# wittyseok/multimodal-organ-segmentation

Hardware: AMD Instinct MI355X
Metric: 96^3 2-modality patches/sec/node (train step) (higher is better)
Workload: dtype bf16; 1 GPU; DualEncoder fusion=cross_attention (mean, dual_encoder.py:193-195) 96^3, modalities CT+PET, 6 classes, DiceCE, AdamW, per-GPU batch 2; model=dual_encoder, global_batch=2, parallelism=dp1, kernels=hip, tag=c3

## Files before the change

multimodal-organ-segmentation_amd/csrc/conv_gemm.hip:

```cpp
#include "mmseg_common.h"

#include <stdlib.h>

#include <algorithm>
#include <type_traits>
#include <cstdio>
#include <vector>

namespace {

int knob(const char* name, int dflt) {
  const char* v = getenv(name);
  return v ? atoi(v) : dflt;
}

enum GatherMode { MODE_CONV3 = 0, MODE_POINT = 1, MODE_CONVT_FWD = 2, MODE_CONVT_DGRAD = 3 };

#ifdef MMSEG_TIMING_PROBES
constexpr int PROBE_NB = 16384;
__device__ long long* g_probe = nullptr;
__device__ __forceinline__ void probe_block(bool end) {
  long long* p = g_probe;
  if (p && threadIdx.x == 0 && blockIdx.x < PROBE_NB) {
    p += 8LL * blockIdx.x;
// ... 1801 lines not shown
  int kind;
  int bz, by, bx;
  int ks;
  int bn;
};

Conv3Plan plan_conv3(int M, int Ncols, int cin, int D, int H, int W, int lda, int ldo, int tsize,
                     bool force_r = false) {
  Conv3Plan p{0, 0, 0, 0, 1, 32};
  bool k1_ok = false;
  const int brick = knob("MMSEG_BRICK", 2);
  const bool base_ok = cin % CK == 0 && lda % 8 == 0 && ldo % 8 == 0 && Ncols % 32 == 0;
  const bool ok48 = cin % CK == 0 && lda % 8 == 0 && ldo % 8 == 0 && Ncols % 48 == 0;
  if (!force_r && brick == 2 && (base_ok || ok48) && D % 4 == 0 && H % B2_Y == 0 && W % B2_X == 0) {
    const long long units = (long long)(M / (D * H * W)) * (D / 4) * (H / B2_Y) * (W / B2_X) *
                            ((Ncols + 63) / 64);
    if (!(base_ok && units < knob("MMSEG_BRICK2_MINUNITS", 128))) {
      p.kind = 1;
      return p;
    }
    k1_ok = true;
  }
  if (brick >= 2 && base_ok) {
    int best = 0;
    for (int bz = 1; bz <= D && bz <= 8; ++bz) {
      if (D % bz) continue;
      for (int by = 1; by <= H && by <= 16; ++by) {
        if (H % by) continue;
        for (int bx = 1; bx <= W && bx <= 16; ++bx) {
          if (W % bx) continue;
          const int rows = bz * by * bx;
          const int halo = (bz + 2) * (by + 2) * (bx + 2);
          const int hq = (bz + 2) * (by + 2) * ((bx + 2) * 2 * tsize + 2);
          if (rows > 256 || halo > BR_MAXHV || hq > br_xq(tsize)) continue;
          const int score = rows * 4 + (bx % 8 == 0 ? 2 : 0) + (by % 8 == 0 ? 1 : 0);
          const bool tie_better = score == best && halo < (p.bz + 2) * (p.by + 2) * (p.bx + 2);
          if (score > best || tie_better) {
            best = score;
            p.bz = bz; p.by = by; p.bx = bx;
          }
        }
      }
    }
    if (best >= 64 * 4) {
      p.kind = 2;
      p.bn = (tsize == 2 && Ncols % 64 == 0) ? 64 : 32;
      const int nb = (M / (D * H * W)) * (D / p.bz) * (H / p.by) * (W / p.bx);
      if (p.bn == 64 && nb * (Ncols / 64) < 256) p.bn = 32;
      const int nt = (Ncols + p.bn - 1) / p.bn;
      const int nchunk = cin / CK;
      const int slots = knob("MMSEG_BRICKR_SLOTS", 256);
      int ks = (slots + nb * nt - 1) / (nb * nt);
      if (ks > nchunk) ks = nchunk;
      if (ks < 1) ks = 1;
      const int cps = (nchunk + ks - 1) / ks;
      p.ks = (nchunk + cps - 1) / cps;
      return p;
    }
  }
  if (k1_ok) p.kind = 1;
  return p;
}

bool brick6_selected(const GemmArgs& g, int tsize) {
  if (tsize != 2 || g.ksplit != 1) return false;
  const Conv3Plan plan = plan_conv3(g.M, g.Ncols, 8 << g.cpg_shift, g.D, g.H, g.W, g.lda, g.ldo, tsize);
  if (plan.kind != 1) return false;
  const int nb1 = (g.M / (g.D * g.H * g.W)) * (g.D / 4) * (g.H / B2_Y) * (g.W / B2_X);
  const int min_blocks = knob("MMSEG_BRICK2_MINBLK", 512);
  const bool v3 = (long long)g.M * g.lda * 2LL < (1LL << 31);
  const bool wide = g.Ncols % 64 == 0 && nb1 * (g.Ncols / 64) >= min_blocks;
  if (!v3 || g.Ncols % 32 != 0 || gemm_nchunk(g) != 1 || wide) return false;
  return g.H % 4 == 0 && g.W % 16 == 0 && g.ldo % 8 == 0 && (reinterpret_cast<uintptr_t>(g.out) & 15) == 0;
}

inline bool tile_in_pitch(const GemmArgs& g, int BN) { return (long long)((g.Ncols + BN - 1) / BN) * BN <= g.Cpad; }
#define MMSEG_TILE(G, NAME, BN)                                                                                   \
  do {                                                                                                           \
    MMSEG_REQUIRE(tile_in_pitch((G), (BN)), "%s: %d-column tiles over %d columns exceed the packed pitch %d", \
                  (const char*)(NAME), (int)(BN), (G).Ncols, (G).Cpad);                                          \
    mmseg::note_kernel(NAME);                                                                                    \
  } while (0)

int launch_brick6(const GemmArgs& g, hipStream_t s) {
  const int nt_n = g.Ncols / 32;
  const int per_nt = std::max(1, knob("MMSEG_BRICK4_BLOCKS", 256) / nt_n);
  const int nb6 = (g.M / (g.D * g.H * g.W)) * (g.D / 4) * (g.H / 4) * (g.W / 16);
  const int upb6 = ceil_div(nb6, std::min(per_nt, nb6));
  const int bpn6 = ceil_div(nb6, upb6);
  const dim3 grid(bpn6 * nt_n), block(256);
  if (g.wdq) {
    MMSEG_TILE(g, "conv3_brick6_kernel<BN32,F8>", 32);
    if (g.nmean) MMSEG_LAUNCH((conv3_brick6_kernel<true, 6, false, true>), grid, block, 0, s, g, upb6, bpn6);
    else MMSEG_LAUNCH((conv3_brick6_kernel<false, 6, false, true>), grid, block, 0, s, g, upb6, bpn6);
    return upb6;
  }
  if (g.inpart) {
    MMSEG_TILE(g, "conv3_brick6_kernel<BN32,INP>", 32);
    MMSEG_LAUNCH((conv3_brick6_kernel<false, 6, true>), grid, block, 0, s, g, upb6, bpn6);
    return upb6;
  }
  MMSEG_TILE(g, "conv3_brick6_kernel<BN32>", 32);
  if (g.nmean)
    MMSEG_LAUNCH((conv3_brick6_kernel<true, 6>), grid, block, 0, s, g, upb6, bpn6);
  else
    MMSEG_LAUNCH((conv3_brick6_kernel<false, 6>), grid, block, 0, s, g, upb6, bpn6);
  return upb6;
}

template <int MODE>
__host__ __device__ __forceinline__ bool splitk_vec(const GemmArgs& g) {
  const bool al = (g.Ncols & 3) == 0 && (g.ldo & 3) == 0 && (reinterpret_cast<uintptr_t>(g.part) & 15) == 0;
  return MODE == MODE_CONVT_FWD ? al && ((g.Ncols >> 3) & 3) == 0 : al;
}
template <int MODE>
int splitk_reduce_blocks(const GemmArgs& g) {
  const long long total = (long long)g.M * g.Ncols;
  return ceil_div(splitk_vec<MODE>(g) ? (total + 3) / 4 : total, 256);
}

template <typename T, int MODE>
__global__ void gemm_splitk_reduce(GemmArgs g) {
  long long total = (long long)g.M * g.Ncols;
  if (MODE == MODE_CONVT_FWD && splitk_vec<MODE>(g)) {
    const long long idx4 = ((long long)blockIdx.x * blockDim.x + threadIdx.x) * 4;
    if (idx4 >= total) return;
    const long long row = idx4 / g.Ncols;
    const int col = (int)(idx4 - row * g.Ncols);
    const int Cout = g.Ncols >> 3, t = col / Cout, co = col - t * Cout;
    float4 v = make_float4(0.f, 0.f, 0.f, 0.f);
    const float4* p = reinterpret_cast<const float4*>(g.part + idx4);
    const long long st = total / 4;
#pragma unroll 4
    for (int k = 0; k < g.ksplit; ++k) {
      const float4 a = p[(long long)k * st];
      v.x += a.x; v.y += a.y; v.z += a.z; v.w += a.w;
    }
    if (g.bias) {
      v.x += g.bias[co]; v.y += g.bias[co + 1]; v.z += g.bias[co + 2]; v.w += g.bias[co + 3];
    }
    T* O = reinterpret_cast<T*>(g.out) + convt_child(row, t, g) * g.ldo + co;
    O[0] = from_f<T>(v.x); O[1] = from_f<T>(v.y); O[2] = from_f<T>(v.z); O[3] = from_f<T>(v.w);
    return;
  }
  if (MODE != MODE_CONVT_FWD && splitk_vec<MODE>(g)) {
    const long long idx4 = ((long long)blockIdx.x * blockDim.x + threadIdx.x) * 4;
    if (idx4 >= total) return;
    const long long row = idx4 / g.Ncols;
    const int col = (int)(idx4 - row * g.Ncols);
    float4 v = make_float4(0.f, 0.f, 0.f, 0.f);
    const float4* p = reinterpret_cast<const float4*>(g.part + idx4);
    const long long st = total / 4;
#pragma unroll 4
    for (int k = 0; k < g.ksplit; ++k) {
      const float4 a = p[(long long)k * st];
      v.x += a.x; v.y += a.y; v.z += a.z; v.w += a.w;
    }
    if (g.bias) {
      const float* bp = g.grp_n > 0 ? g.bias + (int)(row / ((long long)g.D * g.H * g.W) / g.grp_n) * g.b_gstride
                                    : g.bias;
      v.x += bp[col]; v.y += bp[col + 1]; v.z += bp[col + 2]; v.w += bp[col + 3];
    }
    T* O = out_at<T>(g, row, col);
    O[0] = from_f<T>(v.x); O[1] = from_f<T>(v.y); O[2] = from_f<T>(v.z); O[3] = from_f<T>(v.w);
    return;
  }
// ... 1524 lines not shown
      constexpr int PH = decltype(phc)::value;
      if (h_iss < h_tot) {
        issue(h_iss % WROW_NST, dq, du);
        dma_next();
        ++h_iss;
      }
      const char* S = ring + (h % WROW_NST) * WROW_SLOT;
      bf16x8 bfr[WROW_HY];
#pragma unroll
      for (int hy = 0; hy < WROW_HY; ++hy) {
        const bf16_t* pl = reinterpret_cast<const bf16_t*>(S + hy * (WROW_HX * 64) + boff);
        bfr[hy] = tr_frag(pl, pl + 8 * 32);
      }
      const bool anew = u < q.L;
      if (anew) {
#pragma unroll
        for (int r = 0; r < WROW_RY; ++r) {
          const bf16_t* pa = reinterpret_cast<const bf16_t*>(S + r * (32 * 64) + aoff);
          areg[PH][r] = tr_frag(pa, pa + 8 * 32);
        }
      }
      auto mm = [&](auto kzc, const bf16x8(&a)[WROW_RY]) __attribute__((always_inline)) {
        constexpr int KZ = decltype(kzc)::value;
#pragma unroll
        for (int hy = 0; hy < WROW_HY; ++hy)
#pragma unroll
          for (int ky = 0; ky < 3; ++ky) {
            const int ry = hy - ky;
            if (ry >= 0 && ry < WROW_RY)
              acc[KZ][ky] = __builtin_amdgcn_mfma_f32_16x16x32_bf16(a[ry], bfr[hy], acc[KZ][ky], 0, 0, 0);
          }
      };
      if (u >= 2) mm(std::integral_constant<int, 2>{}, areg[(PH + 1) % 3]);
      if (u >= 1 && u <= q.L) mm(std::integral_constant<int, 1>{}, areg[(PH + 2) % 3]);
      if (anew) {
        mm(std::integral_constant<int, 0>{}, areg[PH]);
        if (do_bias && h % 6 == kx * 2 + jh) {
#pragma unroll
          for (int r = 0; r < WROW_RY; ++r) accb = __builtin_amdgcn_mfma_f32_16x16x32_bf16(areg[PH][r], ones, accb, 0, 0, 0);
        }
      }
      wait_cnt(nw * (min(h_tot - 1, h + WROW_NST - 1) - (h + 1)));
      if (h + 1 < h_tot) {
        if (u + 1 < q.L + 2)
          normalize((h + 1) % WROW_NST, q, u + 1);
        else if (q.s + q.L < s_end)
          normalize((h + 1) % WROW_NST, seg_at(q.s + q.L), 0);
      }
      __syncthreads();
      ++h;
    };
    for (int s = s_begin; s < s_end;) {
      const WRowSeg q = seg_at(s);
      for (int u0 = 0; u0 < q.L + 2; u0 += 3) {
        step(std::integral_constant<int, 0>{}, q, u0);
        if (u0 + 1 < q.L + 2) step(std::integral_constant<int, 1>{}, q, u0 + 1);
        if (u0 + 2 < q.L + 2) step(std::integral_constant<int, 2>{}, q, u0 + 2);
      }
      s += q.L;
    }
  }

  float* base = g.part + (long long)ks * g.Ca * g.Ncols + (long long)ct * (32 * 27 * CK);
#pragma unroll
  for (int kz = 0; kz < 3; ++kz)
#pragma unroll
    for (int ky = 0; ky < 3; ++ky) {
      const int tap = kz * 9 + ky * 3 + kx;
      *reinterpret_cast<f32x4*>(base + ((tap * 2 + ih) * 2 + jh) * 256 + lane * 4) = acc[kz][ky];
    }
  if (do_bias) {
    if (i16 == 0) {
#pragma unroll
      for (int r = 0; r < 4; ++r) bred[wave * 16 + 4 * g4 + r] = accb[r];
    }
    __syncthreads();
    if (tid < 32) {
      const int i = tid >> 4;
      float sacc = 0.f;
      for (int w = i; w < WROW_WAVES; w += 2) sacc += bred[w * 16 + (tid & 15)];
      g.bias_part[(long long)ks * g.Ca + tid] = sacc;
    }
  }
}

constexpr int WR_MAXHV = 384;

template <typename T, int MT, int CBZ = 0, int CBY = 0, int CBX = 0>
__global__ __launch_bounds__(512) void wgrad_brickr_kernel(WgradArgs g, int bz_rt, int by_rt, int bx_rt) {
  const int bz = CBZ > 0 ? CBZ : bz_rt, by = CBY > 0 ? CBY : by_rt, bx = CBX > 0 ? CBX : bx_rt;
  constexpr int EP = 16 / sizeof(T);
  constexpr int CO = MT * 16, CG = CO / 8;
  constexpr int DP = CO + EP;
  constexpr int XP = CK + EP;
  constexpr int DS = 128 * DP, XS = WR_MAXHV * XP;
  __shared__ __attribute__((aligned(16))) T lds[2 * (DS + XS)];
  constexpr int D_ITEMS = 128 * CG, X_MAX = WR_MAXHV * 4;
  constexpr int D_PER = (D_ITEMS + 511) / 512, X_PER = (X_MAX + 511) / 512;

  const T* Dy = reinterpret_cast<const T*>(g.a);
  const T* X = reinterpret_cast<const T*>(g.b);
  const int tid = threadIdx.x, lane = tid & 63, wave = tid >> 6;
  const int cin = 8 << g.cpg_shift;
  const int nchunk = wgrad_nchunk(g.cpg_shift, g.kchunks), rt_n = g.Ca / CO;
  const int tile = g.swz ? xcd_swizzle(blockIdx.x, gridDim.x) : (int)blockIdx.x;
  const int ct = tile % nchunk, rt = (tile / nchunk) % rt_n, ks = tile / (nchunk * rt_n);
  const int HX = bx + 2, HY = by + 2, HZ = bz + 2;
  const int HV = HZ * HY * HX, rows = bz * by * bx;
  const int bz_n = g.D / bz, by_n = g.H / by, bx_n = g.W / bx;
  const long long nbrick = (g.V / ((long long)g.D * g.H * g.W)) * bz_n * by_n * bx_n;
  const int ngrp = g.groups > 1 ? g.groups : 1;
  const int ks_g = g.ksplit / ngrp, gi = ks / ks_g, kl = ks - gi * ks_g;
  const long long nb_g = nbrick / ngrp;
  const long long bpk = (nb_g + ks_g - 1) / ks_g;
  const long long b_begin = gi * nb_g + kl * bpk;
  const long long b_end = b_begin + bpk < (gi + 1) * nb_g ? b_begin + bpk : (gi + 1) * nb_g;
  const long long HW = (long long)g.H * g.W;
  const int row0 = rt * CO, c0 = ct * CK;
  const bool do_bias = g.bias_part != nullptr && ct == 0;
  const int t_begin = wave < 3 ? 4 * wave : 12 + 3 * (wave - 3);
  const int t_cnt = wave < 3 ? 4 : 3;

  f32x4 acc[4][MT][2];
#pragma unroll
  for (int t = 0; t < 4; ++t)
#pragma unroll
    for (int i = 0; i < MT; ++i)
#pragma unroll
      for (int j = 0; j < 2; ++j) acc[t][i][j] = (f32x4){0.f, 0.f, 0.f, 0.f};
  float bsum[8] = {0, 0, 0, 0, 0, 0, 0, 0};

  auto vox_halo = [&](int v) {
    if (v >= rows) return 0;
    const int rx = v % bx, q = v / bx;
    return ((q / by) * HY + q % by) * HX + rx;
  };

  V8<T> dr[D_PER], xr[X_PER];
  auto load = [&](long long b) {
    int q = (int)b;
    const int bxi = q % bx_n;
    q /= bx_n;
    const int byi = q % by_n;
    q /= by_n;
    const int bzi = q % bz_n;
    const long long nbase = (long long)(q / bz_n) * g.D * HW;
    const int z0 = bzi * bz, y0 = byi * by, x0 = bxi * bx;
#pragma unroll
    for (int k = 0; k < D_PER; ++k) {
      const int e = tid + k * 512, v = e / CG, cg = e % CG;
      if (e < D_ITEMS) {
        if (v < rows) {
          const int rx = v % bx, qq = v / bx;
          const int ry = qq % by, rz = qq / by;
          dr[k].load(Dy + (nbase + (z0 + rz) * HW + (long long)(y0 + ry) * g.W + x0 + rx) * g.lda + row0 + cg * 8);
        } else {
          dr[k].zero();
        }
      }
    }
#pragma unroll
    for (int k = 0; k < X_PER; ++k) {
      const int e = tid + k * 512;
      if (e < HV * 4) {
        const int h = e >> 2, cg = e & 3;
        const int hx = h % HX, qq = h / HX;
// ... 588 lines not shown
#pragma unroll
      for (int j = 0; j < 8; ++j) w.set(j, s[rr][(cg * 8 + j) * 8 + t]);
      const int co = (k0 >> 3) + cg * 8;
      w.store(dst + ((long long)(t * cpgd + (co >> 3)) * cpad + r0 + rr) * 8);
    }
  }
}

template <typename T>
__global__ __launch_bounds__(256) void adamw_pack_kernel(float* __restrict__ p, const float* __restrict__ g,
                                                         float* __restrict__ m, float* __restrict__ v,
                                                         const AdamPackDesc* __restrict__ descs, int n,
                                                         AdamHyper hv, const AdamHyper* __restrict__ hp,
                                                         const float* __restrict__ skip) {
  __shared__ float sw[8][33][29];
  AdamHyper h;
  if (!adamw_load(hv, hp, skip, h)) return;
  int lo = 0, hi = n - 1;
  const int b = blockIdx.x;
  while (lo < hi) {
    const int mid = (lo + hi + 1) >> 1;
    if (descs[mid].block_begin <= b) lo = mid;
    else hi = mid - 1;
  }
  const AdamPackDesc d = descs[lo];
  const int lb = b - d.block_begin;
  const int tid = threadIdx.x;
  if (d.kind == 0) {
    const int nci = (d.Ci + 31) / 32;
    const int co0 = (lb / nci) * 8, ci0 = (lb % nci) * 32;
    const int cis = d.Ci - ci0 < 32 ? d.Ci - ci0 : 32;
    if (co0 >= d.Co) return;
    for (int e = tid; e < 8 * (32 - cis) * 27; e += 256) {
      const int co = e / ((32 - cis) * 27), r = e - co * ((32 - cis) * 27);
      sw[co][cis + r / 27][r % 27] = 0.f;
    }
    ap_update(p, g, m, v, d.off + ((long long)co0 * d.Ci + ci0) * 27, (long long)d.Ci * 27, 8, cis * 27, h,
              [&](int r, int i, float x) __attribute__((always_inline)) {
                const int ci = i / 27;
                sw[r][ci][i - ci * 27] = x;
              });
    __syncthreads();
    pack3_write<T>(sw, d.d0, d.d1, d.Co, d.Cip, d.Cpad, d.Cpad_d, d.Cop, co0, ci0, cis);
  } else if (d.kind == 1) {
    float (*s)[AP_KT + 1] = reinterpret_cast<float (*)[AP_KT + 1]>(&sw[0][0][0]);
    const int nkt = (d.K + AP_KT - 1) / AP_KT;
    const int r0 = (lb / nkt) * 8, k0 = (lb % nkt) * AP_KT;
    const int kt = d.K - k0 < AP_KT ? d.K - k0 : AP_KT, kt8 = (kt + 7) & ~7;
    if (r0 >= d.R) return;
    for (int e = tid; e < 8 * (kt8 - kt); e += 256) s[e / (kt8 - kt)][kt + e % (kt8 - kt)] = 0.f;
    ap_update(p, g, m, v, d.off + (long long)r0 * d.K + k0, d.K, 8, kt, h,
              [&](int r, int i, float x) __attribute__((always_inline)) { s[r][i] = x; });
    __syncthreads();
    ap_write1<T>(s, d.mode0, d.d0, d.Cpad, d.Co, d.Cop, r0, k0, kt, kt8);
    if (d.d1 != nullptr) ap_write1<T>(s, d.mode1, d.d1, d.Cpad_d, d.Co, d.Cop, r0, k0, kt, kt8);
  } else {
    if (lb * AP_RANGE >= d.K) return;
    const long long a0 = d.off + (long long)lb * AP_RANGE;
    const int len = d.K - lb * AP_RANGE < AP_RANGE ? d.K - lb * AP_RANGE : AP_RANGE;
    ap_update(p, g, m, v, a0, 0, 1, len, h, [](int, int, float) __attribute__((always_inline)) {});
  }
}

template <typename T, int MODE>
int launch_splitk_reduce(const GemmArgs& g, hipStream_t s) {
  const long long total = (long long)g.M * g.Ncols;
  const bool vec = MODE != MODE_CONVT_FWD && splitk_vec<MODE>(g);
  int S = 1;
  while (S < 16 && g.ksplit / (2 * S) >= 4) S *= 2;
  if (vec && S > 1) {
    const int nb = ceil_div(total / 4, 256 / S);
    if (S == 16) MMSEG_LAUNCH((gemm_splitk_reduce_s<T, 16>), dim3(nb), dim3(256), 0, s, g);
    else if (S == 8) MMSEG_LAUNCH((gemm_splitk_reduce_s<T, 8>), dim3(nb), dim3(256), 0, s, g);
    else if (S == 4) MMSEG_LAUNCH((gemm_splitk_reduce_s<T, 4>), dim3(nb), dim3(256), 0, s, g);
    else MMSEG_LAUNCH((gemm_splitk_reduce_s<T, 2>), dim3(nb), dim3(256), 0, s, g);
  } else {
    MMSEG_LAUNCH((gemm_splitk_reduce<T, MODE>), dim3(splitk_reduce_blocks<MODE>(g)), dim3(256), 0, s, g);
  }
  return mmseg::check_launch("gemm_splitk_reduce");
}

template <typename T, int MODE>
int launch_gemm(GemmArgs g, hipStream_t s) {
  if (g.nmean) {
    MMSEG_REQUIRE(MODE == MODE_CONV3 && brick6_selected(g, (int)sizeof(T)),
                  "conv3 with a deferred norm needs the brick6 kernel for this shape (mmseg_conv3_norm_ok)");
    launch_brick6(g, s);
    return mmseg::check_launch("conv3_brick6_norm");
  }
  const int Cbig = g.Ncols >= 64;
  dim3 block(256);
  const int brick = knob("MMSEG_BRICK", 2);
  const Conv3Plan plan = MODE == MODE_CONV3 ? plan_conv3(g.M, g.Ncols, 8 << g.cpg_shift, g.D, g.H, g.W, g.lda, g.ldo,
                                                         (int)sizeof(T), g.grp_n > 0)
                                            : Conv3Plan{0, 0, 0, 0, 1, 32};
  MMSEG_REQUIRE(g.grp_n == 0 || (MODE == MODE_CONV3 && plan.kind == 2),
                "grouped conv: only the runtime-brick kernel takes per-group weights (small volumes)");
  if (plan.kind == 2) {
    const int nb = (g.M / (g.D * g.H * g.W)) * (g.D / plan.bz) * (g.H / plan.by) * (g.W / plan.bx);
    const int nchunk = gemm_nchunk(g);
    if (g.ksplit > nchunk) g.ksplit = nchunk;
    const int cps = (nchunk + g.ksplit - 1) / g.ksplit;
    g.ksplit = (nchunk + cps - 1) / cps;
    const dim3 grid(nb * ((g.Ncols + plan.bn - 1) / plan.bn) * g.ksplit);
    const bool b666 = plan.bz == 6 && plan.by == 6 && plan.bx == 6;
    const bool b488 = plan.bz == 4 && plan.by == 8 && plan.bx == 8;
    const bool rb32 = sizeof(T) == 2 && knob("MMSEG_B32", 1) && (long long)g.M * g.lda * (long long)sizeof(T) < (1LL << 31);
    if (plan.bn == 64) {
      if constexpr (sizeof(T) == 2) {
        MMSEG_TILE(g, "conv3_brickr_kernel<BN64>", 64);
        if (b666 && rb32)
          MMSEG_LAUNCH((conv3_brickr_kernel<T, 64, 6, 6, 6, false, true>), grid, block, 0, s, g, 6, 6, 6);
        else if (b666)
          MMSEG_LAUNCH((conv3_brickr_kernel<T, 64, 6, 6, 6>), grid, block, 0, s, g, 6, 6, 6);
        else if (b488 && rb32)
          MMSEG_LAUNCH((conv3_brickr_kernel<T, 64, 4, 8, 8, false, true>), grid, block, 0, s, g, 4, 8, 8);
        else if (b488)
          MMSEG_LAUNCH((conv3_brickr_kernel<T, 64, 4, 8, 8>), grid, block, 0, s, g, 4, 8, 8);
        else if (rb32)
          MMSEG_LAUNCH((conv3_brickr_kernel<T, 64, 0, 0, 0, false, true>), grid, block, 0, s, g, plan.bz, plan.by,
                       plan.bx);
        else
          MMSEG_LAUNCH((conv3_brickr_kernel<T, 64>), grid, block, 0, s, g, plan.bz, plan.by, plan.bx);
      }
    } else if (b666) {
      const bool kw2 = sizeof(T) == 2 && cps >= 2;
      MMSEG_TILE(g, kw2 ? "conv3_brickr_kernel<BN32,KW2>" : "conv3_brickr_kernel<BN32>", 32);
      bool done = false;
      if constexpr (sizeof(T) == 2) {
        const dim3 b2(512);
        if (kw2 && rb32)
          MMSEG_LAUNCH((conv3_brickr_kernel<T, 32, 6, 6, 6, true, true, 2>), grid, b2, 0, s, g, 6, 6, 6);
        else if (kw2)
          MMSEG_LAUNCH((conv3_brickr_kernel<T, 32, 6, 6, 6, true, false, 2>), grid, b2, 0, s, g, 6, 6, 6);
        done = kw2;
      }
      if (done) {
      } else if (rb32)
        MMSEG_LAUNCH((conv3_brickr_kernel<T, 32, 6, 6, 6, true, true>), grid, block, 0, s, g, 6, 6, 6);
      else
        MMSEG_LAUNCH((conv3_brickr_kernel<T, 32, 6, 6, 6>), grid, block, 0, s, g, 6, 6, 6);
    } else if (b488) {
      MMSEG_TILE(g, "conv3_brickr_kernel<BN32>", 32);
      if (rb32)
        MMSEG_LAUNCH((conv3_brickr_kernel<T, 32, 4, 8, 8, false, true>), grid, block, 0, s, g, 4, 8, 8);
      else
        MMSEG_LAUNCH((conv3_brickr_kernel<T, 32, 4, 8, 8>), grid, block, 0, s, g, 4, 8, 8);
    } else {
      MMSEG_TILE(g, "conv3_brickr_kernel<BN32>", 32);
      if (rb32)
        MMSEG_LAUNCH((conv3_brickr_kernel<T, 32, 0, 0, 0, false, true>), grid, block, 0, s, g, plan.bz, plan.by,
                     plan.bx);
      else
        MMSEG_LAUNCH((conv3_brickr_kernel<T, 32>), grid, block, 0, s, g, plan.bz, plan.by, plan.bx);
    }
    if (mmseg::check_launch("conv3_brickr")) return 1;
    if (g.ksplit > 1) return launch_splitk_reduce<T, MODE>(g, s);
    return 0;
  }
  if (plan.kind == 1 && g.ksplit == 1) {
    const int nb1 = (g.M / (g.D * g.H * g.W)) * (g.D / 4) * (g.H / B2_Y) * (g.W / B2_X);
    const int min_blocks = knob("MMSEG_BRICK2_MINBLK", 512);
    if constexpr (sizeof(T) == 2) {
      const int nb8 = nb1 / 2;
      const int b8 = knob("MMSEG_BRICK8", 1);
      if (b8 && g.Ncols % 64 == 0 && (b8 == 2 || (g.Ncols == 64 && gemm_nchunk(g) >= 2)) && g.D % 8 == 0 &&
          g.H % 8 == 0 && g.W % 8 == 0 &&
          g.nmean == nullptr && g.inpart == nullptr && g.ldo % 8 == 0 &&
          (!g.out2 || g.ldo2 % 8 == 0) && (reinterpret_cast<uintptr_t>(g.out) & 15) == 0 &&
          nb8 * (g.Ncols / 64) >= knob("MMSEG_BRICK8_MINBLK", 256) &&
          (long long)g.M * g.lda * 2 < (1LL << 31) && (long long)((g.KG + 3) & ~3) * g.Cpad * 16 < (1LL << 31)) {
        MMSEG_TILE(g, "conv3_brick8_kernel<BN64>", 64);
        MMSEG_LAUNCH((conv3_brick8_kernel<64, 1>), dim3(nb8 * (g.Ncols / 64)), dim3(512), 0, s, g);
        return mmseg::check_launch("conv3_brick8");
      }
      if (b8 && g.Ncols == 32 && g.D % 16 == 0 && g.H % 8 == 0 && g.W % 8 == 0 &&
          g.nmean == nullptr && g.inpart == nullptr && g.ldo % 8 == 0 &&
          (!g.out2 || g.ldo2 % 8 == 0) && (reinterpret_cast<uintptr_t>(g.out) & 15) == 0 &&
          nb8 / 2 >= knob("MMSEG_BRICK8_MINBLK", 256) && (8 << g.cpg_shift) >= 64 &&
          (long long)g.M * g.lda * 2 < (1LL << 31) && (long long)((g.KG + 3) & ~3) * g.Cpad * 16 < (1LL << 31)) {
        MMSEG_TILE(g, "conv3_brick8_kernel<BN32>", 32);
        MMSEG_LAUNCH((conv3_brick8_kernel<32, 2>), dim3(nb8 / 2), dim3(512), 0, s, g);
        return mmseg::check_launch("conv3_brick8");
      }
    }
    const bool v3 = sizeof(T) == 2 && (long long)g.M * g.lda * (long long)sizeof(T) < (1LL << 31);
    const int maxblk = knob("MMSEG_BRICK3_BLOCKS", 512);
    const bool b32 = sizeof(T) == 2 && knob("MMSEG_B32", 1) && (long long)g.M * g.lda * (long long)sizeof(T) < (1LL << 31);
    const bool wide = g.Ncols % 64 == 0 && nb1 * (g.Ncols / 64) >= min_blocks;
    const bool bn48 = g.Ncols % 32 != 0 || (g.Ncols % 96 == 0 && g.Ncols % 64 != 0);
    if (bn48) {
      MMSEG_TILE(g, "conv3_brick2_kernel<BN48,ZW1>", 48);
      if (b32) {
        MMSEG_LAUNCH((conv3_brick2_kernel<T, 48, 1, false, true>), dim3(nb1 * (g.Ncols / 48)), block, 0, s, g);
        return mmseg::check_launch("conv3_brick2");
      }
      MMSEG_LAUNCH((conv3_brick2_kernel<T, 48, 1>), dim3(nb1 * (g.Ncols / 48)), block, 0, s, g);
    } else if (v3 && gemm_nchunk(g) == 1 && g.Ncols % 32 == 0 && !wide) {
      if constexpr (sizeof(T) == 2) {
        const int nt_n = g.Ncols / 32;
        const int per_nt = std::max(1, knob("MMSEG_BRICK4_BLOCKS", 256) / nt_n);
        const int upb = ceil_div(nb1, std::min(per_nt, nb1));
        const int bpn = ceil_div(nb1, upb);
        if (g.H % 4 == 0 && g.W % 16 == 0 && g.ldo % 8 == 0 && (reinterpret_cast<uintptr_t>(g.out) & 15) == 0) {
          launch_brick6(g, s);
        } else {
          MMSEG_TILE(g, "conv3_brick4_kernel<BN32>", 32);
          MMSEG_LAUNCH(conv3_brick4_kernel, dim3(bpn * nt_n), block, 0, s, g, upb, bpn);
        }
      }
    } else if (v3 && !wide) {
      const int units = nb1 * (g.Ncols / 32);
      const int upb = maxblk > 0 ? ceil_div(units, maxblk) : 1;
      MMSEG_TILE(g, "conv3_brick3_kernel<BN32>", 32);
      MMSEG_LAUNCH((conv3_brick3_kernel<T, 32>), dim3(ceil_div(units, upb)), block, 0, s, g, upb);
    } else if (wide) {
      MMSEG_TILE(g, "conv3_brick2_kernel<BN64,ZW1>", 64);
      if (b32)
        MMSEG_LAUNCH((conv3_brick2_kernel<T, 64, 1, true, true>), dim3(nb1 * (g.Ncols / 64)), block, 0, s, g);
      else
        MMSEG_LAUNCH((conv3_brick2_kernel<T, 64, 1, true>), dim3(nb1 * (g.Ncols / 64)), block, 0, s, g);
    } else {
      MMSEG_TILE(g, "conv3_brick2_kernel<BN32,ZW1>", 32);
      MMSEG_LAUNCH((conv3_brick2_kernel<T, 32, 1>), dim3(nb1 * (g.Ncols / 32)), block, 0, s, g);
    }
    return mmseg::check_launch("conv3_brick2");
  }
  if (MODE == MODE_CONV3 && g.ksplit == 1 && brick == 1 && (8 << g.cpg_shift) % CK == 0 &&
      g.D % BRK_Z == 0 && g.H % BRK_Y == 0 && g.W % BRK_X == 0 && g.lda % 8 == 0) {
    const int nb = (g.M / (g.D * g.H * g.W)) * (g.D / BRK_Z) * (g.H / BRK_Y) * (g.W / BRK_X);
    const int bn = g.Ncols >= 64 ? 64 : 32;
    MMSEG_TILE(g, bn == 64 ? "conv3_brick_kernel<BN64>" : "conv3_brick_kernel<BN32>", bn);
    if (bn == 64) {
      MMSEG_LAUNCH((conv3_brick_kernel<T, 64>), dim3(nb * ceil_div(g.Ncols, 64)), block, 0, s, g);
    } else {
      MMSEG_LAUNCH((conv3_brick_kernel<T, 32>), dim3(nb * ceil_div(g.Ncols, 32)), block, 0, s, g);
    }
    return mmseg::check_launch("conv3_brick");
  }
  if (MODE == MODE_CONVT_FWD && g.Ncols % 256 == 0) {
    MMSEG_TILE(g, "conv_gemm_kernel<convT_fwd,64x256>", 256);
    dim3 grid(ceil_div(g.M, 64) * (g.Ncols / 256) * g.ksplit);
    MMSEG_LAUNCH((conv_gemm_kernel<T, MODE, 1, 4, 4, 4>), grid, block, 0, s, g);
    if (mmseg::check_launch("conv_gemm")) return 1;
    if (g.ksplit > 1) return launch_splitk_reduce<T, MODE>(g, s);
    return 0;
  }
  if (MODE == MODE_POINT && g.ksplit == 1 && g.Ncols > 128 && g.Ncols <= 192 && g.Cpad >= 192) {
    if constexpr (MODE == MODE_POINT) {
      MMSEG_TILE(g, "conv_gemm_kernel<point,64x192>", 192);
      dim3 grid(ceil_div(g.M, 64));
      MMSEG_LAUNCH((conv_gemm_kernel<T, MODE, 1, 4, 4, 3>), grid, block, 0, s, g);
    }
  } else if (MODE == MODE_POINT && g.ksplit == 1 && g.Ncols > 64 && g.Ncols <= 128 && g.Ncols % 96 != 0) {
    if constexpr (MODE == MODE_POINT) {
      MMSEG_TILE(g, "conv_gemm_kernel<point,64x128>", 128);
      dim3 grid(ceil_div(g.M, 64));
      MMSEG_LAUNCH((conv_gemm_kernel<T, MODE, 1, 4, 4, 2>), grid, block, 0, s, g);
    }
  } else if (MODE == MODE_POINT && g.ksplit == 1 && g.Ncols > 32 && g.Ncols <= 48 && g.Ncols % 16 == 0) {
    if constexpr (MODE == MODE_POINT) {
      MMSEG_TILE(g, "conv_gemm_kernel<point,128x48>", 48);
      dim3 grid(ceil_div(g.M, 128));
      MMSEG_LAUNCH((conv_gemm_kernel<T, MODE, 4, 1, 2, 3>), grid, block, 0, s, g);
    }
  } else if (MODE == MODE_POINT && g.Ncols % 96 == 0 && g.Ncols % 64 != 0) {
    if constexpr (MODE == MODE_POINT) {
      MMSEG_TILE(g, "conv_gemm_kernel<point,128x96>", 96);
      dim3 grid(ceil_div(g.M, 128) * (g.Ncols / 96) * g.ksplit);
      MMSEG_LAUNCH((conv_gemm_kernel<T, MODE, 2, 2, 4, 3>), grid, block, 0, s, g);
    }
  } else if (!Cbig) {
    static const char* nm[4] = {"conv_gemm_kernel<conv3,128x32>", "conv_gemm_kernel<point,128x32>",
                                "conv_gemm_kernel<convT_fwd,128x32>", "conv_gemm_kernel<convT_dgrad,128x32>"};
    MMSEG_TILE(g, nm[MODE], 32);
    dim3 grid(ceil_div(g.M, 128) * ceil_div(g.Ncols, 32) * g.ksplit);
    MMSEG_LAUNCH((conv_gemm_kernel<T, MODE, 4, 1, 2, 2>), grid, block, 0, s, g);
  } else {
    static const char* nm[4] = {"conv_gemm_kernel<conv3,128x64>", "conv_gemm_kernel<point,128x64>",
                                "conv_gemm_kernel<convT_fwd,128x64>", "conv_gemm_kernel<convT_dgrad,128x64>"};
    MMSEG_TILE(g, nm[MODE], 64);
    dim3 grid(ceil_div(g.M, 128) * ceil_div(g.Ncols, 64) * g.ksplit);
    MMSEG_LAUNCH((conv_gemm_kernel<T, MODE, 2, 2, 4, 2>), grid, block, 0, s, g);
  }
  if (mmseg::check_launch("conv_gemm")) return 1;
  if (g.ksplit > 1) return launch_splitk_reduce<T, MODE>(g, s);
  return 0;
// ... 405 lines not shown
  const int KGp = (KG + 3) & ~3;
  GemmArgs g{a, lda, wpacked, bias, out, ldo, nullptr, M, Ncols, Cpad, KG, 0, 1, 1, 1, 1, KGp,
             1 , 0, nullptr, nullptr};
  MMSEG_REQUIRE(lda % 8 == 0, "conv_gemm_gelu: lda must be a multiple of 8");
  MMSEG_REQUIRE(Cpad >= ((Ncols + (Ncols >= 64 ? 63 : 31)) / (Ncols >= 64 ? 64 : 32)) * (Ncols >= 64 ? 64 : 32),
                "conv_gemm_gelu: packed weights must be padded to the column tile (Cpad=%d, Ncols=%d)", Cpad, Ncols);
  g.epi = epi;
  g.aux = gelu_in;
  g.aux_out = gelu_out;
  hipStream_t s = (hipStream_t)stream;
  if (dtype == MMSEG_BF16) return launch_gemm<bf16_t, MODE_POINT>(g, s);
  return launch_gemm<float, MODE_POINT>(g, s);
}

int mmseg_conv_gemm_res(const void* a, int lda, const void* wpacked, const float* bias, const void* res, int ldres,
                        void* out, int ldo, int M, int Ncols, int Cpad, int KG, int dtype, void* stream) {
  MMSEG_REQUIRE(res != nullptr, "conv_gemm_res: residual required");
  return conv_gemm_impl(a, lda, wpacked, bias, out, ldo, nullptr, 0, 0, nullptr, MODE_POINT, M, Ncols, Cpad, KG, 0, 1,
                        1, 1, 1, 0, dtype, stream, 1, 0, 0, res, ldres);
}

int mmseg_conv_gemm_split(const void* a, int lda, const void* wpacked, const float* bias, void* out, int ldo,
                          void* out2, int ldo2, int split, float* splitk_ws, int mode, int M, int Ncols, int Cpad,
                          int KG, int cpg_shift, int D, int H, int W, int ksplit, int cin_real, int dtype,
                          void* stream) {
  MMSEG_REQUIRE(out2 && split > 0 && split < Ncols && split % 8 == 0 && ldo2 % 8 == 0 && ldo % 8 == 0 &&
                    (reinterpret_cast<uintptr_t>(out2) & 15) == 0 && mode != MODE_CONVT_FWD,
                "conv_gemm_split: split %d must be a multiple of 8 inside (0, %d), ldo / ldo2 multiples of 8, out2 "
                "16-B aligned", split, Ncols);
  return conv_gemm_impl(a, lda, wpacked, bias, out, ldo, out2, ldo2, split, splitk_ws, mode, M, Ncols, Cpad, KG,
                        cpg_shift, D, H, W, ksplit, cin_real, dtype, stream);
}

int conv_gemm_impl(const void* a, int lda, const void* wpacked, const float* bias, void* out, int ldo, void* out2,
                   int ldo2, int split, float* splitk_ws, int mode, int M, int Ncols, int Cpad, int KG, int cpg_shift,
                   int D, int H, int W, int ksplit, int cin_real, int dtype, void* stream, int groups,
                   long long w_gstride, int b_gstride, const void* res, int ldres, int zcols) {
  MMSEG_REQUIRE(zcols == 0 || (zcols >= Ncols && zcols % 8 == 0 && zcols <= ldo && !out2 && Ncols % 8 == 0 &&
                               zcols - Ncols <= 48),
                "conv_gemm: whole-row extent zcols=%d must lie in [Ncols, min(ldo, Ncols + 48)]", zcols);
  MMSEG_REQUIRE(!res || (mode == MODE_POINT && ksplit == 1 && !out2 && ldo % 8 == 0 && ldres % 8 == 0 &&
                         Ncols % 8 == 0 && ((reinterpret_cast<uintptr_t>(out) | reinterpret_cast<uintptr_t>(res)) &
                                            15) == 0),
                "conv_gemm_res: MODE_POINT, ksplit 1, pitches and Ncols multiples of 8, 16-B aligned out / res");
  MMSEG_REQUIRE(cin_real >= 0 && cin_real <= (8 << cpg_shift), "conv_gemm: cin_real %d outside [0, %d]", cin_real,
                8 << cpg_shift);
  MMSEG_REQUIRE(lda % 8 == 0 && ldo >= 1, "conv_gemm: lda must be a multiple of 8 (got %d)", lda);
  MMSEG_REQUIRE(Cpad >= ((Ncols + (Ncols >= 64 ? 63 : 31)) / (Ncols >= 64 ? 64 : 32)) * (Ncols >= 64 ? 64 : 32),
                "conv_gemm: packed weights must be padded to the column tile (Cpad=%d, Ncols=%d)", Cpad, Ncols);
  MMSEG_REQUIRE(ksplit >= 1, "conv_gemm: ksplit >= 1");
  MMSEG_REQUIRE(ksplit == 1 || splitk_ws != nullptr, "conv_gemm: split-K needs a workspace");
  const int KGp = (KG + 3) & ~3;
  int kps = ((ceil_div(KGp, ksplit) + 3) / 4) * 4;
  ksplit = ceil_div(KGp, kps);
  GemmArgs g{a, lda, wpacked, bias, out, ldo, splitk_ws, M, Ncols, Cpad, KG, cpg_shift, D, H, W, ksplit, kps,
             1 , mode == MODE_CONV3 ? (cin_real + 31) / 32 : 0, nullptr, nullptr, out2, ldo2,
             split};
  if (groups > 1) {
    g.grp_n = M / (D * H * W) / groups;
    g.w_gstride = w_gstride;
    g.b_gstride = b_gstride;
  }
  g.res = res;
  g.ldres = ldres;
  g.zcols = zcols;
  hipStream_t s = (hipStream_t)stream;
  if (dtype == MMSEG_BF16) return launch_gemm_mode<bf16_t>(g, mode, s);
  return launch_gemm_mode<float>(g, mode, s);
}

int mmseg_conv3_norm_ok(int M, int Ncols, int Cpad, int KG, int cpg_shift, int D, int H, int W, int lda, int ldo,
                        int dtype) {
  if (dtype != MMSEG_BF16 || !knob("MMSEG_DEFER_CONV_NORM", 1)) return 0;
  GemmArgs g{};
  g.lda = lda; g.ldo = ldo; g.M = M; g.Ncols = Ncols; g.Cpad = Cpad; g.KG = KG; g.cpg_shift = cpg_shift;
  g.D = D; g.H = H; g.W = W; g.ksplit = 1;
  g.out = reinterpret_cast<void*>(static_cast<uintptr_t>(256));
  return brick6_selected(g, 2) ? 1 : 0;
}

int mmseg_conv3_fwd_norm(const void* a, int lda, const float* nmean, const float* nrstd, const void* wpacked,
                         const float* bias, void* out, int ldo, int M, int Ncols, int Cpad, int KG, int cpg_shift,
                         int D, int H, int W, int dtype, void* stream) {
  MMSEG_REQUIRE(nmean && nrstd && (reinterpret_cast<uintptr_t>(out) & 15) == 0 &&
                    mmseg_conv3_norm_ok(M, Ncols, Cpad, KG, cpg_shift, D, H, W, lda, ldo, dtype),
                "conv3_fwd_norm: unsupported shape (mmseg_conv3_norm_ok)");
  const int KGp = (KG + 3) & ~3;
  GemmArgs g{a, lda, wpacked, bias, out, ldo, nullptr, M, Ncols, Cpad, KG, cpg_shift, D, H, W, 1, KGp,
             1 , 0, nmean, nrstd};
  return launch_gemm<bf16_t, MODE_CONV3>(g, (hipStream_t)stream);
}

int mmseg_conv3_fp8_ok(int M, int Ncols, int Cpad, int KG, int cpg_shift, int D, int H, int W, int lda, int ldo) {
  GemmArgs g{};
  g.lda = lda; g.ldo = ldo; g.M = M; g.Ncols = Ncols; g.Cpad = Cpad; g.KG = KG; g.cpg_shift = cpg_shift;
  g.D = D; g.H = H; g.W = W; g.ksplit = 1;
  g.out = reinterpret_cast<void*>(static_cast<uintptr_t>(256));
  return brick6_selected(g, 2) ? 1 : 0;
}

int mmseg_pack_conv3_fp8(const float* w, int Co, int Ci, int Cip, int KGp, int Cpad, void* dst, float* wdq,
                         void* stream) {
  MMSEG_REQUIRE(w && dst && wdq && Co > 0 && Co <= Cpad && Ci <= Cip && Cip % 8 == 0 && KGp * 8 >= 27 * Cip,
                "pack_conv3_fp8: bad arguments");
  hipStream_t s = (hipStream_t)stream;
  hipMemsetAsync(dst, 0, (size_t)KGp * Cpad * 8, s);
  MMSEG_LAUNCH(pack_conv3_fp8_kernel, dim3(Co), dim3(256), 0, s, w, Ci, Cip, Cpad, (unsigned char*)dst, wdq);
  return mmseg::check_launch("pack_conv3_fp8");
}

int mmseg_conv3_fwd_fp8(const void* a, int lda, const float* nmean, const float* nrstd, const void* w8,
                        const float* wdq, const float* bias, void* out, int ldo, int M, int Ncols, int Cpad, int KG,
                        int cpg_shift, int D, int H, int W, void* stream) {
  MMSEG_REQUIRE(a && w8 && wdq && out && (nmean == nullptr) == (nrstd == nullptr) &&
                    (reinterpret_cast<uintptr_t>(out) & 15) == 0 &&
                    mmseg_conv3_fp8_ok(M, Ncols, Cpad, KG, cpg_shift, D, H, W, lda, ldo),
                "conv3_fwd_fp8: unsupported shape (mmseg_conv3_fp8_ok)");
  const int KGp = (KG + 3) & ~3;
  GemmArgs g{a, lda, w8, bias, out, ldo, nullptr, M, Ncols, Cpad, KG, cpg_shift, D, H, W, 1, KGp,
             1 , 0, nmean, nrstd};
  g.wdq = wdq;
  launch_brick6(g, (hipStream_t)stream);
  return mmseg::check_launch("conv3_fwd_fp8");
}

int mmseg_conv3_dgrad_in_chunks(int M, int Ncols, int Cpad, int KG, int cpg_shift, int D, int H, int W, int lda,
                                int ldo, int dtype) {
  if (dtype != MMSEG_BF16) return 0;
  GemmArgs g{};
  g.lda = lda; g.ldo = ldo; g.M = M; g.Ncols = Ncols; g.Cpad = Cpad; g.KG = KG; g.cpg_shift = cpg_shift;
  g.D = D; g.H = H; g.W = W; g.ksplit = 1;
  g.out = reinterpret_cast<void*>(static_cast<uintptr_t>(256));
  if (!brick6_selected(g, 2)) return 0;
  const int nt_n = Ncols / 32;
  const int per_nt = std::max(1, knob("MMSEG_BRICK4_BLOCKS", 256) / nt_n);
  const int nb6 = (M / (D * H * W)) * (D / 4) * (H / 4) * (W / 16);
  const int upb6 = ceil_div(nb6, std::min(per_nt, nb6));
  return ceil_div(nb6, upb6);
}

int mmseg_conv3_dgrad_in(const void* a, int lda, const void* wpacked, void* out, int ldo, int M, int Ncols, int Cpad,
                         int KG, int cpg_shift, int D, int H, int W, const void* inx, int ldinx, const float* inmean,
                         const float* inrstd, float* inpart, int dtype, void* stream) {
  MMSEG_REQUIRE(inx && inmean && inrstd && inpart && ldinx % 8 == 0 && (reinterpret_cast<uintptr_t>(out) & 15) == 0 &&
                    mmseg_conv3_dgrad_in_chunks(M, Ncols, Cpad, KG, cpg_shift, D, H, W, lda, ldo, dtype) > 0,
                "conv3_dgrad_in: unsupported shape (mmseg_conv3_dgrad_in_chunks)");
  const int KGp = (KG + 3) & ~3;
  GemmArgs g{a, lda, wpacked, nullptr, out, ldo, nullptr, M, Ncols, Cpad, KG, cpg_shift, D, H, W, 1, KGp,
             1 , 0, nullptr, nullptr};
  g.inx = inx;
  g.ldinx = ldinx;
  g.inmean = inmean;
  g.inrstd = inrstd;
  g.inpart = inpart;
  launch_brick6(g, (hipStream_t)stream);
  return mmseg::check_launch("conv3_dgrad_in");
}

int mmseg_conv3_group_ok(int M, int Ncols, int Cpad, int KG, int cpg_shift, int D, int H, int W, int lda, int ldo,
                         int dtype) {
  if (!knob("MMSEG_GROUP_SMALL", 1)) return 0;
  const int ts = dtype == MMSEG_BF16 ? 2 : 4;
  if (plan_conv3(M, Ncols, 8 << cpg_shift, D, H, W, lda, ldo, ts).kind == 2) return 1;
  return knob("MMSEG_GROUP_FORCE_R", 1) && plan_conv3(M, Ncols, 8 << cpg_shift, D, H, W, lda, ldo, ts, true).kind == 2
             ? 1 : 0;
}
int mmseg_conv3_wgrad_group_ok(long long V, int Co, int Cip, int Ci, int cpg_shift, int D, int H, int W, int lddy,
                               int ldx, int dtype) {
  if (!knob("MMSEG_GROUP_SMALL", 1)) return 0;
  if (plan_conv3_wgrad(V, Co, Cip, Ci, cpg_shift, D, H, W, lddy, ldx, dtype, 1LL << 40).kind == 3) return 1;
  return knob("MMSEG_GROUP_FORCE_R", 1) &&
                 plan_conv3_wgrad(V, Co, Cip, Ci, cpg_shift, D, H, W, lddy, ldx, dtype, 1LL << 40, true).kind == 3
// ... 272 lines not shown
```

Measured before the change: 343.3 patches/s.

## Add row-streaming conv3 kernel with LDS ring and z-sliding accumulators

Adds a new 3x3x3 conv forward kernel for 32-output-channel bf16 layers. Each block streams z-planes of an input row strip through a multi-stage LDS ring using async DMA, and keeps weights resident in registers. Three rotating accumulators let each loaded plane feed all three kz taps, and the deferred norm+ReLU is applied in LDS. By default it replaces brick6 for the deferred-norm path. It aims to cut redundant halo loads and overlap memory with MFMA, at the cost of high register/LDS use and one block per CU.

After: 343.9 patches/s, median of 3. Within noise of the previous version (+0.2%).

```diff
diff --git a/multimodal-organ-segmentation_amd/csrc/conv_gemm.hip b/multimodal-organ-segmentation_amd/csrc/conv_gemm.hip
--- a/multimodal-organ-segmentation_amd/csrc/conv_gemm.hip
+++ b/multimodal-organ-segmentation_amd/csrc/conv_gemm.hip
@@ -1907,6 +1907,10 @@
     mmseg::note_kernel(NAME);                                                                                    \
   } while (0)
 
+bool conv3_row_ok(const GemmArgs& g);
+bool conv3_row_forced(const GemmArgs& g);
+int launch_conv3_row(const GemmArgs& g, hipStream_t s);
+
 int launch_brick6(const GemmArgs& g, hipStream_t s) {
   const int nt_n = g.Ncols / 32;
   const int per_nt = std::max(1, knob("MMSEG_BRICK4_BLOCKS", 256) / nt_n);
@@ -3597,6 +3601,313 @@
       g.bias_part[(long long)ks * g.Ca + tid] = sacc;
     }
   }
+}
+
+template <int RY>
+struct CRowGeo {
+  static constexpr int HY = RY + 2;
+  static constexpr int NW = 2 * RY;
+  static constexpr int HI = (HY * WROW_HX * 4 + 63) / 64;
+  static constexpr int KI = (HI + NW - 1) / NW;
+  static constexpr int SLOT = HI * 1024;
+};
+
+template <bool NORM, int RY = 6, int NST = 4>
+__global__ __launch_bounds__(128 * RY, 1) void conv3_row_kernel(GemmArgs g, int spb) {
+  typedef __attribute__((address_space(3))) void* lds_ptr_t;
+  typedef __bf16 bf16x4 __attribute__((ext_vector_type(4)));
+  typedef CRowGeo<RY> G;
+  constexpr int HY = G::HY, NW = G::NW, HI = G::HI, KI = G::KI, SLOT = G::SLOT;
+  constexpr int ROWB = WROW_HX * 64;
+  __shared__ __attribute__((aligned(16))) char ring[NST * SLOT];
+  __shared__ __attribute__((aligned(16))) float ntab[NORM ? 2 * WROW_MAXN * 32 : 4];
+  __shared__ __attribute__((aligned(16))) float btab[32];
+
+  const int tid = threadIdx.x, lane = tid & 63, wave = __builtin_amdgcn_readfirstlane(tid >> 6);
+  const int ry = wave >> 1, j = wave & 1;
+  const int r16 = lane & 15, kg = lane >> 4;
+  const int cin = 8 << g.cpg_shift;
+  const int D = g.D, H = g.H, W = g.W;
+  const int ncx = W / 32, ncol = (H / RY) * ncx;
+  const int N = g.M / (D * H * W);
+  const int s_tot = N * ncol * D;
+  const int blk = g.swz ? xcd_swizzle(blockIdx.x, gridDim.x) : (int)blockIdx.x;
+  const int s_begin = min(blk * spb, s_tot), s_end = min(s_begin + spb, s_tot);
+  if (s_begin >= s_end) return;
+  const wd_rsrc_t arsrc = wd_rsrc(g.a, (uint32_t)((long long)g.M * g.lda * 2));
+
+  bf16x8 wf[27];
+  {
+    const bf16_t* Bw = reinterpret_cast<const bf16_t*>(g.b);
+#pragma unroll
+    for (int t = 0; t < 27; ++t)
+      wf[t] = *reinterpret_cast<const bf16x8*>(
+          Bw + ((long long)(t * (cin / 8) + kg) * g.Cpad + 8 * (r16 >> 2) + 4 * j + (r16 & 3)) * 8);
+  }
+  if (tid < 32) btab[tid] = g.bias ? g.bias[tid] : 0.f;
+
+  auto seg_at = [&](int s) __attribute__((always_inline)) {
+    WRowSeg q;
+    q.s = s;
+    q.col = s / D;
+    q.za = s - q.col * D;
+    q.L = min(D, s_end - q.col * D) - q.za;
+    return q;
+  };
+  int h_tot = 0;
+  for (int s = s_begin; s < s_end;) {
+    const WRowSeg q = seg_at(s);
+    h_tot += q.L + 2;
+    s += q.L;
+  }
+
+  int nw = 0;
+  int pos[KI];
+#pragma unroll
+  for (int k = 0; k < KI; ++k) {
+    const int m = wave + NW * k;
+    pos[k] = 0xff;
+    if (m < HI) {
+      const int p = m * 64 + lane, hy = p / (WROW_HX * 4), r = p - hy * (WROW_HX * 4), xh = r >> 2, cs = r & 3;
+      const int cc = cs ^ (((xh >> 2) & 1) << 1);
+      if (hy < HY) pos[k] = hy | (xh << 8) | (cc << 16);
+      ++nw;
+    }
+  }
+  struct ColPos { int n, y0, x0; };
+  auto col_pos = [&](int col) __attribute__((always_inline)) {
+    ColPos c;
+    c.n = col / ncol;
+    const int cr = col - c.n * ncol, by = cr / ncx;
+    c.y0 = by * RY;
+    c.x0 = (cr - by * ncx) * 32;
+    return c;
+  };
+  auto issue = [&](int slot, const WRowSeg& q, const ColPos& c, int u) __attribute__((always_inline)) {
+    const int zh = q.za - 1 + u;
+    const bool zh_ok = (unsigned)zh < (unsigned)D;
+    const int hb = (((c.n * D + zh) * H + (c.y0 - 1)) * W + (c.x0 - 1)) * g.lda * 2;
+    const uint32_t lbase = (uint32_t)(uintptr_t)(lds_ptr_t)(ring + slot * SLOT);
+#pragma unroll
+    for (int k = 0; k < KI; ++k) {
+      const int m = wave + NW * k;
+      if (m < HI) {
+        int pk = pos[k];
+        asm volatile("" : "+v"(pk));
+        const int py = pk & 0xff, xh = (pk >> 8) & 0xff, y = c.y0 - 1 + py, x = c.x0 - 1 + xh;
+        const bool ok = zh_ok && py != 0xff && (unsigned)y < (unsigned)H && (unsigned)x < (unsigned)W;
+        const int rel = ((py * W + xh) * g.lda + (pk >> 16) * 8) * 2;
+        wd_dma16(__builtin_amdgcn_readfirstlane(lbase + m * 1024), ok ? (uint32_t)(hb + rel) : WD_OOB, arsrc);
+      }
+    }
+  };
+  auto wait_cnt = [&](int cnt) __attribute__((always_inline)) {
+    switch (cnt) {
+#define MMSEG_CR_WAIT(N) \
+  case N: __builtin_amdgcn_s_waitcnt(0x0f70 | N); break;
+      MMSEG_CR_WAIT(1) MMSEG_CR_WAIT(2) MMSEG_CR_WAIT(3) MMSEG_CR_WAIT(4) MMSEG_CR_WAIT(5) MMSEG_CR_WAIT(6)
+      MMSEG_CR_WAIT(7) MMSEG_CR_WAIT(8) MMSEG_CR_WAIT(9) MMSEG_CR_WAIT(10) MMSEG_CR_WAIT(11) MMSEG_CR_WAIT(12)
+      MMSEG_CR_WAIT(13) MMSEG_CR_WAIT(14) MMSEG_CR_WAIT(15)
+#undef MMSEG_CR_WAIT
+      default: __builtin_amdgcn_s_waitcnt(0x0f70); break;
+    }
+  };
+  auto normalize = [&](int slot, const WRowSeg& q, const ColPos& c, int u) __attribute__((always_inline)) {
+    if constexpr (NORM) {
+      const int zh = q.za - 1 + u;
+      if ((unsigned)zh >= (unsigned)D) return;
+#pragma unroll
+      for (int k = 0; k < KI; ++k) {
+        const int m = wave + NW * k;
+        if (m < HI) {
+          int pk = pos[k];
+          asm volatile("" : "+v"(pk));
+          const int py = pk & 0xff, y = c.y0 - 1 + py, x = c.x0 - 1 + ((pk >> 8) & 0xff), cc = pk >> 16;
+          if (py != 0xff && (unsigned)y < (unsigned)H && (unsigned)x < (unsigned)W) {
+            bf16_t* p = reinterpret_cast<bf16_t*>(ring + slot * SLOT + m * 1024 + (threadIdx.x & 63) * 16);
+            const float4* mu4 = reinterpret_cast<const float4*>(ntab + c.n * 32 + cc * 8);
+            const float4* rs4 = reinterpret_cast<const float4*>(ntab + WROW_MAXN * 32 + c.n * 32 + cc * 8);
+            bf16x8 v = *reinterpret_cast<const bf16x8*>(p);
+#pragma unroll
+            for (int hf = 0; hf < 2; ++hf) {
+              const float4 m4 = mu4[hf], r4 = rs4[hf];
+              const float mu[4] = {m4.x, m4.y, m4.z, m4.w}, rs[4] = {r4.x, r4.y, r4.z, r4.w};
+#pragma unroll
+              for (int e = 0; e < 4; ++e) {
+                const float hv = ((float)v[4 * hf + e] - mu[e]) * rs[e];
+                v[4 * hf + e] = (bf16_t)(hv > 0.f ? hv : 0.f);
+              }
+            }
+            *reinterpret_cast<bf16x8*>(p) = v;
+          }
+        }
+      }
+    }
+  };
+
+  int fo[3];
+#pragma unroll
+  for (int kx = 0; kx < 3; ++kx) {
+    const int hx = r16 + kx;
+    fo[kx] = ry * ROWB + hx * 64 + 16 * (kg ^ (((hx >> 2) & 1) << 1));
+  }
+  const int ooff = r16 * g.ldo + 8 * kg + 4 * j;
+  f32x4 acc[3][2];
+#pragma unroll
+  for (int a = 0; a < 3; ++a)
+#pragma unroll
+    for (int b = 0; b < 2; ++b) acc[a][b] = (f32x4){0.f, 0.f, 0.f, 0.f};
+
+  if constexpr (NORM) {
+    for (int e = tid; e < N * 32; e += NW * 64) {
+      const int n = e >> 5, c = e & 31;
+      ntab[n * 32 + c] = g.nmean[n * cin + c];
+      ntab[WROW_MAXN * 32 + n * 32 + c] = g.nrstd[n * cin + c];
+    }
+  }
+  __syncthreads();
+  WRowSeg dq = seg_at(s_begin);
+  ColPos dc = col_pos(dq.col);
+  int du = 0;
+  auto dma_next = [&]() __attribute__((always_inline)) {
+    if (++du == dq.L + 2) {
+      du = 0;
+      if (dq.s + dq.L < s_end) {
+        dq = seg_at(dq.s + dq.L);
+        dc = col_pos(dq.col);
+      }
+    }
+  };
+  int h_iss = 0;
+  for (; h_iss < NST - 1 && h_iss < h_tot; ++h_iss) {
+    issue(h_iss % NST, dq, dc, du);
+    dma_next();
+  }
+  wait_cnt(nw * (min(h_tot - 1, NST - 2)));
+  normalize(0, seg_at(s_begin), col_pos(s_begin / D), 0);
+  __syncthreads();
+
+  int h = 0;
+  int st1 = 0, st2 = 0;
+  auto step = [&](auto phc, const WRowSeg& q, const ColPos& c, int u) __attribute__((always_inline)) {
+    constexpr int PH = decltype(phc)::value;
+    if (h_iss < h_tot) {
+      issue(h_iss % NST, dq, dc, du);
+      dma_next();
+      ++h_iss;
+    }
+    const char* S = ring + (h % NST) * SLOT;
+    auto frag = [&](int kx, int ky, int xr) __attribute__((always_inline)) {
+      return *reinterpret_cast<const bf16x8*>(S + fo[kx] + ky * ROWB + xr * 1024);
+    };
+    const f32x4 zero = {0.f, 0.f, 0.f, 0.f};
+    const bool k2 = u >= 2, k1 = u >= 1 && u <= q.L, k0 = u < q.L;
+    if (k2 && k1 && k0) {
+      constexpr int PFD = 2;
+      bf16x8 fr[PFD + 1];
+#pragma unroll
+      for (int f = 0; f < PFD; ++f) fr[f] = frag(f / 6, (f / 2) % 3, f & 1);
+#pragma unroll
+      for (int f = 0; f < 18; ++f) {
+        const int kx = f / 6, ky = (f / 2) % 3, xr = f & 1;
+        if (f + PFD < 18) fr[(f + PFD) % (PFD + 1)] = frag((f + PFD) / 6, ((f + PFD) / 2) % 3, (f + PFD) & 1);
+        const bf16x8 a = fr[f % (PFD + 1)];
+        acc[(PH + 1) % 3][xr] =
+            __builtin_amdgcn_mfma_f32_16x16x32_bf16(wf[18 + ky * 3 + kx], a, acc[(PH + 1) % 3][xr], 0, 0, 0);
+        acc[(PH + 2) % 3][xr] =
+            __builtin_amdgcn_mfma_f32_16x16x32_bf16(wf[9 + ky * 3 + kx], a, acc[(PH + 2) % 3][xr], 0, 0, 0);
+        acc[PH][xr] = __builtin_amdgcn_mfma_f32_16x16x32_bf16(wf[ky * 3 + kx], a, f < 2 ? zero : acc[PH][xr], 0, 0, 0);
+        __builtin_amdgcn_sched_barrier(0);
+      }
+    } else {
+      auto mm = [&](auto kzc, f32x4(&a)[2]) __attribute__((always_inline)) {
+        constexpr int KZ = decltype(kzc)::value;
+#pragma unroll
+        for (int kx = 0; kx < 3; ++kx)
+#pragma unroll
+          for (int ky = 0; ky < 3; ++ky) {
+#pragma unroll
+            for (int xr = 0; xr < 2; ++xr)
+              a[xr] = __builtin_amdgcn_mfma_f32_16x16x32_bf16(wf[KZ * 9 + ky * 3 + kx], frag(kx, ky, xr),
+                                                              KZ == 0 && kx == 0 && ky == 0 ? zero : a[xr], 0, 0, 0);
+            __builtin_amdgcn_sched_barrier(0);
+          }
+      };
+      if (k2) mm(std::integral_constant<int, 2>{}, acc[(PH + 1) % 3]);
+      if (k1) mm(std::integral_constant<int, 1>{}, acc[(PH + 2) % 3]);
+      if (k0) mm(std::integral_constant<int, 0>{}, acc[PH]);
+    }
+    int st0 = 0;
+    if (k2) {
+      const int z = q.za + u - 2;
+      bf16_t* O = reinterpret_cast<bf16_t*>(g.out) +
+                  ((long long)((c.n * D + z) * H + c.y0 + ry) * W + c.x0) * g.ldo + ooff;
+      const float4 bv = *reinterpret_cast<const float4*>(btab + 8 * ((threadIdx.x >> 4) & 3) + 4 * j);
+      const float bvr[4] = {bv.x, bv.y, bv.z, bv.w};
+#pragma unroll
+      for (int xr = 0; xr < 2; ++xr) {
+        bf16x4 o;
+#pragma unroll
+        for (int r = 0; r < 4; ++r) o[r] = (bf16_t)(acc[(PH + 1) % 3][xr][r] + bvr[r]);
+        *reinterpret_cast<bf16x4*>(O + (long long)(16 * xr) * g.ldo) = o;
+      }
+      st0 = 2;
+    }
+    asm volatile("" ::: "memory");
+    wait_cnt(nw * (min(h_tot - 1, h + NST - 1) - (h + 1)) + st0 + st1 + st2);
+    st2 = st1;
+    st1 = st0;
+    if (h + 1 < h_tot) {
+      if (u + 1 < q.L + 2) {
+        normalize((h + 1) % NST, q, c, u + 1);
+      } else if (q.s + q.L < s_end) {
+        const WRowSeg qn = seg_at(q.s + q.L);
+        normalize((h + 1) % NST, qn, col_pos(qn.col), 0);
+      }
+    }
+    __syncthreads();
+    ++h;
+  };
+  for (int s = s_begin; s < s_end;) {
+    const WRowSeg q = seg_at(s);
+    const ColPos c = col_pos(q.col);
+    for (int u0 = 0; u0 < q.L + 2; u0 += 3) {
+      step(std::integral_constant<int, 0>{}, q, c, u0);
+      if (u0 + 1 < q.L + 2) step(std::integral_constant<int, 1>{}, q, c, u0 + 1);
+      if (u0 + 2 < q.L + 2) step(std::integral_constant<int, 2>{}, q, c, u0 + 2);
+    }
+    s += q.L;
+  }
+}
+
+bool conv3_row_ok(const GemmArgs& g) {
+  const int mode = knob("MMSEG_CONV_ROW", 1);
+  if (mode <= 0 || (mode == 1 && !g.nmean)) return false;
+  if (g.wdq || g.inpart || g.grp_n || g.out2 || g.res || g.epi || g.ksplit != 1) return false;
+  const long long vox = (long long)g.D * g.H * g.W;
+  return gemm_nchunk(g) == 1 && g.Ncols == 32 && g.W % 32 == 0 && g.H % 4 == 0 && g.lda % 8 == 0 &&
+         g.ldo % 8 == 0 && (reinterpret_cast<uintptr_t>(g.a) & 15) == 0 &&
+         (reinterpret_cast<uintptr_t>(g.out) & 15) == 0 && (long long)g.M * g.lda * 2 < (1LL << 31) &&
+         (long long)((g.KG + 3) & ~3) * g.Cpad * 16 < (1LL << 31) && g.M / vox <= WROW_MAXN;
+}
+
+bool conv3_row_forced(const GemmArgs& g) { return knob("MMSEG_CONV_ROW", 1) == 3 && conv3_row_ok(g); }
+
+int launch_conv3_row(const GemmArgs& g, hipStream_t s) {
+  const int ry = g.H % 6 == 0 ? 6 : 4;
+  const int s_tot = (g.M / (g.D * g.H * g.W)) * (g.H / ry) * (g.W / 32) * g.D;
+  const int nblk = std::max(1, std::min(knob("MMSEG_BRICK4_BLOCKS", 256), s_tot));
+  const int spb = ceil_div(s_tot, nblk);
+  const dim3 grid(ceil_div(s_tot, spb));
+  MMSEG_TILE(g, "conv3_row_kernel<BN32>", 32);
+  if (g.nmean) {
+    if (ry == 6) MMSEG_LAUNCH((conv3_row_kernel<true, 6>), grid, dim3(768), 0, s, g, spb);
+    else MMSEG_LAUNCH((conv3_row_kernel<true, 4>), grid, dim3(512), 0, s, g, spb);
+  } else {
+    if (ry == 6) MMSEG_LAUNCH((conv3_row_kernel<false, 6>), grid, dim3(768), 0, s, g, spb);
+    else MMSEG_LAUNCH((conv3_row_kernel<false, 4>), grid, dim3(512), 0, s, g, spb);
+  }
+  return 0;
 }
 
 constexpr int WR_MAXHV = 384;
@@ -4351,9 +4662,19 @@
 
 template <typename T, int MODE>
 int launch_gemm(GemmArgs g, hipStream_t s) {
+  if constexpr (MODE == MODE_CONV3 && sizeof(T) == 2) {
+    if (conv3_row_forced(g)) {
+      if (launch_conv3_row(g, s)) return 1;
+      return mmseg::check_launch("conv3_row");
+    }
+  }
   if (g.nmean) {
     MMSEG_REQUIRE(MODE == MODE_CONV3 && brick6_selected(g, (int)sizeof(T)),
                   "conv3 with a deferred norm needs the brick6 kernel for this shape (mmseg_conv3_norm_ok)");
+    if (conv3_row_ok(g)) {
+      if (launch_conv3_row(g, s)) return 1;
+      return mmseg::check_launch("conv3_row_norm");
+    }
     launch_brick6(g, s);
     return mmseg::check_launch("conv3_brick6_norm");
   }
@@ -4472,6 +4793,10 @@
         const int upb = ceil_div(nb1, std::min(per_nt, nb1));
         const int bpn = ceil_div(nb1, upb);
         if (g.H % 4 == 0 && g.W % 16 == 0 && g.ldo % 8 == 0 && (reinterpret_cast<uintptr_t>(g.out) & 15) == 0) {
+          if (conv3_row_ok(g)) {
+            if (launch_conv3_row(g, s)) return 1;
+            return mmseg::check_launch("conv3_row");
+          }
           launch_brick6(g, s);
         } else {
           MMSEG_TILE(g, "conv3_brick4_kernel<BN32>", 32);
@@ -5043,12 +5368,13 @@
 int mmseg_conv3_fwd_norm(const void* a, int lda, const float* nmean, const float* nrstd, const void* wpacked,
                          const float* bias, void* out, int ldo, int M, int Ncols, int Cpad, int KG, int cpg_shift,
                          int D, int H, int W, int dtype, void* stream) {
-  MMSEG_REQUIRE(nmean && nrstd && (reinterpret_cast<uintptr_t>(out) & 15) == 0 &&
-                    mmseg_conv3_norm_ok(M, Ncols, Cpad, KG, cpg_shift, D, H, W, lda, ldo, dtype),
-                "conv3_fwd_norm: unsupported shape (mmseg_conv3_norm_ok)");
   const int KGp = (KG + 3) & ~3;
   GemmArgs g{a, lda, wpacked, bias, out, ldo, nullptr, M, Ncols, Cpad, KG, cpg_shift, D, H, W, 1, KGp,
              1 , 0, nmean, nrstd};
+  MMSEG_REQUIRE(nmean && nrstd && (reinterpret_cast<uintptr_t>(out) & 15) == 0 &&
+                    (mmseg_conv3_norm_ok(M, Ncols, Cpad, KG, cpg_shift, D, H, W, lda, ldo, dtype) ||
+                     (dtype == MMSEG_BF16 && conv3_row_forced(g))),
+                "conv3_fwd_norm: unsupported shape (mmseg_conv3_norm_ok)");
   return launch_gemm<bf16_t, MODE_CONV3>(g, (hipStream_t)stream);
 }
 
```
